# Zelana-Labs/zelana

Hardware: AMD Instinct MI355X
Metric: BN254 G1 MSM Mpoint-scalar/s + L2 proofs/sec at 1/2/4/8 MI355X (higher is better)
Workload: dtype u32

## Files before the change

zelana_amd/csrc/msm.hip:

```cpp
#include <stdarg.h>
#include <stdlib.h>
#include <stdio.h>
#include <string.h>

#include <algorithm>
#include <string>
#include <type_traits>
#include <vector>
#include <chrono>

#include "dev_io.h"
#include "ec.h"
#include "zkmi_internal.h"

namespace zk {

#define ZK_TAIL_WAVE() __builtin_amdgcn_s_setprio(3)

struct G1T {
  using F = FqOps;
  using P = FqP;
  static constexpr int CW = 8;
  static constexpr int PW = 16;
};
// ... 153 lines not shown
  extern __shared__ uint32_t hist[];
  for (uint32_t x = threadIdx.x; x < NH; x += RS_THREADS) hist[x] = 0;
  __syncthreads();
  const uint64_t base = (uint64_t)blockIdx.x * C1;
  const double inv_ne = 1.0 / (double)ne;
  constexpr int U = 8;
  for (uint32_t k0 = 0; k0 < C1; k0 += U * RS_THREADS) {
    int32_t d[U];
#pragma unroll
    for (int u = 0; u < U; u++) {
      uint64_t e = base + k0 + u * RS_THREADS + threadIdx.x;
      d[u] = (k0 + u * RS_THREADS + threadIdx.x < C1 && e < M) ? digits[e] : 0;
    }
#pragma unroll
    for (int u = 0; u < U; u++) {
      if (d[u] == 0) continue;
      uint32_t w, i;
      rs_divmod(base + k0 + u * RS_THREADS + threadIdx.x, ne, inv_ne, w, i);
      atomicAdd(&hist[(w * B + (uint32_t)(d[u] < 0 ? -d[u] : d[u]) - 1) >> lob], 1u);
    }
  }
  __syncthreads();
  for (uint32_t x = threadIdx.x; x < NH; x += RS_THREADS) cnt1[(size_t)x * nc1 + blockIdx.x] = hist[x];
}


template <int T = RS_THREADS>
__device__ __forceinline__ uint32_t rs_block_scan(const uint32_t* hist, uint32_t* lstart, uint32_t nb, uint32_t* tmp) {
  uint32_t sum = 0;
  for (uint32_t x = threadIdx.x; x < nb; x += T) sum += hist[x];
  const uint32_t lane = threadIdx.x & 63, wid = threadIdx.x >> 6;
  uint32_t inc = sum;
#pragma unroll
  for (int off = 1; off < 64; off <<= 1) {
    uint32_t t = __shfl_up(inc, off, 64);
    if (lane >= (unsigned)off) inc += t;
  }
  if (lane == 63) tmp[wid] = inc;
  __syncthreads();
  uint32_t run = inc - sum, total = 0;
#pragma unroll
  for (int w = 0; w < T / 64; w++) {
    const uint32_t tw = tmp[w];
    if ((uint32_t)w < wid) run += tw;
    total += tw;
  }
  for (uint32_t x = threadIdx.x; x < nb; x += T) {
    lstart[x] = run;
    run += hist[x];
  }
  return total;
}

template <int PER, class Fill, class Bin, bool WRITE_KEY, int T = RS_THREADS, class KT = uint32_t>
__device__ __forceinline__ void rs_scatter_core(uint32_t nsub, uint32_t nb, uint32_t* lds, Fill fill, Bin bin,
                                                 KT* __restrict__ okey, uint32_t* __restrict__ oval) {
  uint32_t* hist = lds;
  uint32_t* lstart = lds + nb;
  uint32_t* gbase = lds + 2 * nb;
  uint32_t* tmp = lds + 3 * nb;
  uint32_t* skey = tmp + T;
  uint32_t* sval = skey + PER * T;
  for (uint32_t x = threadIdx.x; x < nb; x += T) hist[x] = 0;
  __syncthreads();
  for (uint32_t sub = 0; sub < nsub; sub++) {
    uint32_t key[PER], val[PER], rk[PER];
    bool ok[PER];
    fill(sub, key, val, ok);
#pragma unroll
    for (int k = 0; k < PER; k++)
      if (ok[k]) rk[k] = atomicAdd(&hist[bin(key[k])], 1u);
    __syncthreads();
    const uint32_t total = rs_block_scan<T>(hist, lstart, nb, tmp);
    __syncthreads();
#pragma unroll
    for (int k = 0; k < PER; k++) {
      if (ok[k]) {
        uint32_t lp = lstart[bin(key[k])] + rk[k];
        skey[lp] = key[k];
        sval[lp] = val[k];
      }
    }
    __syncthreads();
    for (uint32_t q = threadIdx.x; q < total; q += T) {
      uint32_t kk = skey[q], bn = bin(kk);
      uint32_t g = gbase[bn] + (q - lstart[bn]);
      if (WRITE_KEY) okey[g] = (KT)kk;
      oval[g] = sval[q];
    }
    __syncthreads();
    for (uint32_t x = threadIdx.x; x < nb; x += T) {
      gbase[x] += hist[x];
      hist[x] = 0;
    }
    __syncthreads();
  }
}

template <int RS_ST, class Load, class Bin, bool WRITE_KEY, int T = RS_THREADS>
__device__ __forceinline__ void rs_scatter_tiles(uint32_t count, uint32_t nb, uint32_t* lds, Load load, Bin bin,
                                                 uint32_t* __restrict__ okey, uint32_t* __restrict__ oval) {
  constexpr int PER = RS_ST / T;
  auto fill = [&](uint32_t sub, uint32_t* key, uint32_t* val, bool* ok) {
#pragma unroll
    for (int k = 0; k < PER; k++) {
      const uint32_t e = sub * RS_ST + k * T + threadIdx.x;
      ok[k] = e < count && load(e, key[k], val[k]);
    }
  };
  rs_scatter_core<PER, decltype(fill), Bin, WRITE_KEY, T>((count + RS_ST - 1) / RS_ST, nb, lds, fill, bin, okey, oval);
}

__host__ __device__ constexpr size_t rs_scatter_lds(uint32_t nb, uint32_t st, uint32_t t = RS_THREADS) {
  return (3 * (size_t)nb + t + 2 * st) * 4;
}

template <int RS_ST>
__global__ void __launch_bounds__(RS_THREADS) k_rs_p1_scatter(const int32_t* __restrict__ digits, uint64_t M,
                                                              uint32_t ne, uint32_t B, uint32_t NH, uint32_t lob,
                                                              uint32_t C1, uint32_t nc1, const uint32_t* __restrict__ offs1,
                                                              uint32_t* __restrict__ okey, uint32_t* __restrict__ oval) {
  ZK_TAIL_WAVE();
  extern __shared__ uint32_t lds[];
  for (uint32_t x = threadIdx.x; x < NH; x += RS_THREADS) lds[2 * NH + x] = offs1[(size_t)x * nc1 + blockIdx.x];
  const uint64_t base = (uint64_t)blockIdx.x * C1;
  const uint32_t count = (uint32_t)std::min<uint64_t>(C1, M - base);
  auto load = [&](uint32_t e, uint32_t& key, uint32_t& val) { return rs_key(digits, base + e, ne, B, key, val); };
  auto bin = [lob](uint32_t key) { return key >> lob; };
  rs_scatter_tiles<RS_ST, decltype(load), decltype(bin), true>(count, NH, lds, load, bin, okey, oval);
}

template <int C, bool BAL>
__device__ __forceinline__ void rs_scalar_keys(const uint32_t* __restrict__ scalars, size_t i, size_t n, int Wp,
                                               uint32_t B, uint32_t* key, uint32_t* val, bool* ok, uint32_t wsel) {
  constexpr int W = msm_windows(C);
  int32_t d[W];
  scalar_digits<C, BAL>(scalars, i, d);
  const uint32_t w0 = wsel & 0xFFFFu, wn = wsel >> 16;
  uint32_t j = 0, wq = 0;
#pragma unroll
  for (int w = 0; w < W; w++) {
    const int32_t v = d[w];
    const uint32_t wr = (uint32_t)w - w0;
    ok[w] = v != 0 && (wn == 0 || wr < wn);
    key[w] = (wn ? wr : wq) * B + (uint32_t)(v < 0 ? -v : v) - 1;
    val[w] = (uint32_t)(j * n + i) | (v < 0 ? 0x80000000u : 0u);
    if (++wq == (uint32_t)Wp) {
      wq = 0;
      j++;
    }
  }
}

constexpr size_t SMALL_SORT_MAX = (size_t)1 << 18;
template <int C, bool BAL, bool BAT = false>
__global__ void __launch_bounds__(256) k_ss_count(const uint32_t* __restrict__ scalars, size_t n, int Wp, uint32_t B,
                                                  uint32_t wsel, uint32_t* __restrict__ cnt, size_t sstride = 0) {
  ZK_TAIL_WAVE();
  constexpr int W = msm_windows(C);
  const size_t i = blockIdx.x * (size_t)blockDim.x + threadIdx.x;
  if (i >= n) return;
  uint32_t key[W], val[W];
  bool ok[W];
  if (BAT) scalars += (size_t)blockIdx.y * sstride;
  rs_scalar_keys<C, BAL>(scalars, i, n, Wp, B, key, val, ok, wsel);
  const uint32_t koff = BAT ? blockIdx.y * (uint32_t)Wp * B : 0u;
#pragma unroll
// ... 246 lines not shown
template <int C, int T, bool BAL, bool BAT = false>
__global__ void __launch_bounds__(T) k_bs_scatter1(const uint32_t* __restrict__ scalars, size_t n, int Wp, uint32_t B,
                                                   uint32_t wsel, uint32_t NH, uint32_t lob, uint32_t CS, uint32_t scs,
                                                   const uint32_t* __restrict__ bintot,
                                                   const uint32_t* __restrict__ sctot,
                                                   const uint32_t* __restrict__ choff, BsKey* __restrict__ okey,
                                                   uint32_t* __restrict__ oval, uint32_t nfb = 0, size_t sstride = 0) {
  ZK_TAIL_WAVE();
  extern __shared__ uint32_t lds[];
  constexpr int W = msm_windows(C);
  uint32_t* gbase = lds + 2 * NH;
  block_prefix<T>(NH, [&](uint32_t k) { return bintot[k]; }, gbase, lds + 3 * NH);
  const uint32_t s0 = blockIdx.x >> scs;
  for (uint32_t x = threadIdx.x; x < NH; x += T) {
    uint32_t g = gbase[x] + choff[(size_t)blockIdx.x * NH + x];
    for (uint32_t q = 0; q < s0; q++) g += sctot[(size_t)q * NH + x];
    gbase[x] = g;
  }
  const uint32_t bq = BAT ? blockIdx.x / nfb : 0u;
  const size_t base = (size_t)(BAT ? blockIdx.x - bq * nfb : blockIdx.x) * CS;
  const uint32_t cnt = (uint32_t)std::min<size_t>(CS, n - base);
  const uint32_t koff = BAT ? bq * (uint32_t)Wp * B : 0u;
  if (BAT) scalars += (size_t)bq * sstride;
  auto fill = [&](uint32_t sub, uint32_t* key, uint32_t* val, bool* ok) {
    const uint32_t k = sub * T + threadIdx.x;
    if (k < cnt) {
      rs_scalar_keys<C, BAL>(scalars, base + k, n, Wp, B, key, val, ok, wsel);
      if (BAT) {
#pragma unroll
        for (int w = 0; w < W; w++) key[w] += koff;
      }
    } else {
#pragma unroll
      for (int w = 0; w < W; w++) ok[w] = false;
    }
  };
  auto bin = [lob](uint32_t key) { return key >> lob; };
  rs_scatter_core<W, decltype(fill), decltype(bin), true, T>((cnt + T - 1) / T, NH, lds, fill, bin, okey, oval);
}

__device__ __forceinline__ uint32_t bs_tiles(const uint32_t* __restrict__ bintot, uint32_t NH, uint32_t C2,
                                             uint32_t* pre, uint32_t* tst, uint32_t* tmp) {
  const uint32_t M = block_prefix<256>(NH, [&](uint32_t k) { return bintot[k]; }, pre, tmp);
  const uint32_t TT = block_prefix<256>(
      NH, [&](uint32_t k) { return max(1u, (bintot[k] + C2 - 1) / C2); }, tst, tmp);
  if (threadIdx.x == 0) {
    pre[NH] = M;
    tst[NH] = TT;
  }
  __syncthreads();
  return TT;
}

__global__ void __launch_bounds__(256) k_bs_count2(const BsKey* __restrict__ okey,
                                                   const uint32_t* __restrict__ bintot, uint32_t NH, uint32_t lob,
                                                   uint32_t C2, uint32_t T2max, uint32_t* __restrict__ thist) {
  ZK_TAIL_WAVE();
  extern __shared__ uint32_t lds[];
  const uint32_t NLO = 1u << lob, mask = NLO - 1;
  uint32_t* hist = lds;
  uint32_t* pre = lds + NLO;
  uint32_t* tst = pre + NH + 1;
  uint32_t* tmp = tst + NH + 1;
  const uint32_t t = rs_xcd_tile(blockIdx.x, T2max);
  if (t >= T2max) return;
  const uint32_t TT = bs_tiles(bintot, NH, C2, pre, tst, tmp);
  if (t >= TT) return;
  const uint32_t h = rs_tile_bin(tst, NH, t), q = t - tst[h];
  const uint32_t lo = pre[h] + q * C2, hi = min(lo + C2, pre[h + 1]);
  for (uint32_t x = threadIdx.x; x < NLO; x += 256) hist[x] = 0;
  __syncthreads();
  constexpr int U = 8;
  for (uint32_t p0 = lo; p0 < hi; p0 += U * 256) {
    uint32_t kk[U];
#pragma unroll
    for (int u = 0; u < U; u++) {
      const uint32_t p = p0 + u * 256 + threadIdx.x;
      kk[u] = p < hi ? okey[p] : 0xFFFFFFFFu;
    }
#pragma unroll
    for (int u = 0; u < U; u++)
      if (kk[u] != 0xFFFFFFFFu) atomicAdd(&hist[kk[u] & mask], 1u);
  }
  __syncthreads();
  for (uint32_t x = threadIdx.x; x < NLO; x += 256) thist[(size_t)t * NLO + x] = hist[x];
}

struct ItemsOut {
  uint4* items;
  uint32_t nmain, cap;
  uint32_t* itc;
  uint4* split;
  uint4* stage;
  uint32_t* ghist;
};

template <int ST, bool ITEMS>
__global__ void __launch_bounds__(256) k_bs_scatter2(const BsKey* __restrict__ okey,
                                                     const uint32_t* __restrict__ oval,
                                                     const uint32_t* __restrict__ bintot, uint32_t NH, uint32_t lob,
                                                     uint32_t C2, uint32_t T2max, uint32_t K,
                                                     const uint32_t* __restrict__ thist,
                                                     uint32_t* __restrict__ sval, uint32_t* __restrict__ bstart,
                                                     ItemsOut io) {
  ZK_TAIL_WAVE();
  constexpr int T = 256;
  extern __shared__ uint32_t lds[];
  const uint32_t NLO = 1u << lob, mask = NLO - 1;
  uint32_t* lstart = lds + NLO;
  uint32_t* gbase = lds + 2 * NLO;
  uint32_t* tmp = lds + 3 * NLO;
  uint32_t* skey = tmp + T;
  uint32_t* pre = skey + 2 * ST;
  uint32_t* tst = pre + NH + 1;
  const uint32_t t = rs_xcd_tile(blockIdx.x, T2max);
  if (t >= T2max) return;
  const uint32_t TT = bs_tiles(bintot, NH, C2, pre, tst, tmp);
  if (t >= TT) return;
  const uint32_t h = rs_tile_bin(tst, NH, t), q = t - tst[h];
  const uint32_t lo = pre[h] + q * C2, hi = min(lo + C2, pre[h + 1]);
  const uint32_t k0 = h * NLO;
  uint32_t* ksz = lds;
  {
    const uint32_t t0 = tst[h], nt = tst[h + 1] - t0;
    for (uint32_t x = threadIdx.x; x < NLO; x += T) {
      uint32_t tot = 0, before = 0;
      for (uint32_t qq = 0; qq < nt; qq++) {
        const uint32_t v = thist[(size_t)(t0 + qq) * NLO + x];
        before += qq < q ? v : 0u;
        tot += v;
      }
      ksz[x] = k0 + x < K ? tot : 0u;
      gbase[x] = before;
    }
    __syncthreads();
  }
  auto ksize = [&](uint32_t x) { return ksz[x]; };
  block_prefix<T>(NLO, ksize, lstart, tmp);
  if (q == 0) {
    for (uint32_t x = threadIdx.x; x < NLO; x += T)
      if (k0 + x < K) bstart[k0 + x] = pre[h] + lstart[x];
    if (h == NH - 1 && threadIdx.x == 0) bstart[K] = pre[NH];
    if constexpr (ITEMS) {
      const uint32_t cap = io.cap;
      uint32_t* ch = skey;
      uint32_t* cstart = skey + ST;
      for (uint32_t c = threadIdx.x; c <= cap; c += T) ch[c] = 0;
      __syncthreads();
      constexpr uint32_t PERX = 2048 / T;
      uint32_t tk[PERX];
#pragma unroll
      for (uint32_t j = 0; j < PERX; j++) {
        const uint32_t x = j * T + threadIdx.x;
        if (x < NLO) tk[j] = atomicAdd(&ch[min(ksize(x), cap)], 1u);
      }
      __syncthreads();
      block_prefix<T>(cap + 1, [&](uint32_t k) { return ch[cap - k]; }, cstart, tmp);
#pragma unroll
      for (uint32_t j = 0; j < PERX; j++) {
        const uint32_t x = j * T + threadIdx.x;
        if (x >= NLO) continue;
        const uint32_t size = ksize(x), cls = min(size, cap);
        const uint32_t rank = cstart[cap - cls] + tk[j];
        const uint32_t start = pre[h] + lstart[x];
        const uint32_t np = (size + cap - 1) / cap;
        uint32_t slot0 = 0xFFFFFFFFu;
        if (np > 1) {
          slot0 = atomicAdd(&io.itc[1], np);
          const uint32_t ov = atomicAdd(&io.itc[0], np - 1);
          io.split[atomicAdd(&io.itc[2], 1u)] = make_uint4(k0 + x, slot0, np, 0);
          for (uint32_t pc = 1; pc < np; pc++)
            io.items[io.nmain + ov + pc - 1] =
                make_uint4(start + pc * cap, min(start + (pc + 1) * cap, start + size), k0 + x, slot0 + pc);
        }
        io.stage[(size_t)h * NLO + rank] = make_uint4(start, start + cls, k0 + x, slot0);
      }
      for (uint32_t c = threadIdx.x; c <= cap; c += T)
        if (ch[c]) atomicAdd(&io.ghist[c], ch[c]);
      __syncthreads();
    }
  }
  for (uint32_t x = threadIdx.x; x < NLO; x += T) gbase[x] += pre[h] + lstart[x];
  auto load = [&](uint32_t e, uint32_t& key, uint32_t& val) {
    key = okey[lo + e];
    val = oval[lo + e];
    return true;
  };
  auto bin = [mask](uint32_t key) { return key & mask; };
  rs_scatter_tiles<ST, decltype(load), decltype(bin), false, T>(hi - lo, NLO, lds, load, bin, nullptr, sval);
}

__global__ void __launch_bounds__(256) k_scan_blocks(const uint32_t* in, uint32_t K, uint32_t* out,
                                                     uint32_t* __restrict__ block_sums) {
  ZK_TAIL_WAVE();
  __shared__ uint32_t sh[256];
  uint32_t base = blockIdx.x * 1024 + threadIdx.x * 4;
  uint32_t v[4], s = 0;
#pragma unroll
  for (int k = 0; k < 4; k++) {
    v[k] = base + k < K ? in[base + k] : 0;
    s += v[k];
  }
  sh[threadIdx.x] = s;
  __syncthreads();
  for (int off = 1; off < 256; off <<= 1) {
    uint32_t t = threadIdx.x >= (unsigned)off ? sh[threadIdx.x - off] : 0;
    __syncthreads();
    sh[threadIdx.x] += t;
    __syncthreads();
  }
  uint32_t excl = sh[threadIdx.x] - s;
#pragma unroll
  for (int k = 0; k < 4; k++) {
    if (base + k < K) out[base + k] = excl;
    excl += v[k];
  }
  if (threadIdx.x == 255) block_sums[blockIdx.x] = sh[255];
}
__global__ void __launch_bounds__(1024) k_scan_top(uint32_t* __restrict__ bs, uint32_t nb, uint32_t* __restrict__ total) {
  ZK_TAIL_WAVE();
  __shared__ uint32_t sh[1024];
  uint32_t carry = 0;
  for (uint32_t base = 0; base < nb; base += 1024) {
    uint32_t i = base + threadIdx.x;
    uint32_t v = i < nb ? bs[i] : 0;
    sh[threadIdx.x] = v;
    __syncthreads();
    for (int off = 1; off < 1024; off <<= 1) {
      uint32_t t = threadIdx.x >= (unsigned)off ? sh[threadIdx.x - off] : 0;
      __syncthreads();
      sh[threadIdx.x] += t;
      __syncthreads();
    }
    if (i < nb) bs[i] = sh[threadIdx.x] - v + carry;
    uint32_t blk_total = sh[1023];
    __syncthreads();
    carry += blk_total;
  }
  if (threadIdx.x == 0) *total = carry;
}
__global__ void __launch_bounds__(256) k_scan_add(uint32_t* __restrict__ out, uint32_t K,
                                                  const uint32_t* __restrict__ bs, uint32_t* __restrict__ cursor) {
// ... 1497 lines not shown
  uint32_t B, K;
  int w0 = 0;
  uint32_t wsel = 0;
  int nb = 1;
  bool batch = false;
  size_t sstride = 0;
  int Wp() const { return wsel ? msm_windows(c) : W / nb; }
};
static MsmPlan msm_plan(const zkmi_ctx* ctx, const zkmi_bases* tb, size_t n) {
  MsmPlan P;
  const bool table = tb->tc > 0 && (ctx->msm_window == 0 || ctx->msm_window == tb->tc);
  P.c = table ? tb->tc : (ctx->msm_window > 0 ? ctx->msm_window : pick_window(n));
  P.p = table ? tb->tp : 1;
  P.W = table ? tb->tw : msm_windows(P.c);
  P.bal = table && tb->tbal;
  P.ne = (size_t)P.p * n;
  P.Mmax = (size_t)P.W * P.ne;
  P.B = 1u << (P.c - 1);
  P.K = (uint32_t)P.W * P.B;
  P.bb = P.c - 1;
  P.lb = (P.bb + 1) / 2;
  P.hb = P.bb - P.lb;
  return P;
}
static MsmPlan msm_plan_batch(const zkmi_ctx* ctx, const zkmi_bases* tb, size_t n, int nb, size_t sstride) {
  MsmPlan P = msm_plan(ctx, tb, n);
  P.batch = true;
  P.nb = nb;
  P.sstride = sstride;
  P.W *= nb;
  P.K *= (uint32_t)nb;
  P.Mmax *= (size_t)nb;
  return P;
}
static bool same_plan(const MsmPlan& a, const MsmPlan& b) {
  return a.c == b.c && a.p == b.p && a.W == b.W && a.bal == b.bal;
}
static bool items_plan(const MsmPlan& P) {
  return P.K >= ITEMS_MIN_K && P.c >= 12 && P.c <= 22 && (P.W <= 2 || P.Mmax <= (size_t)64 * P.K);
}
static uint32_t item_cap(const zkmi_ctx* ctx, const MsmPlan& P) {
  const size_t share = P.Mmax / ((size_t)ctx->num_cus * 768 * 2);
  uint32_t cap = 64;
  while (cap < share && cap < ITEM_CAP_MAX) cap <<= 1;
  return cap;
}
struct BsGeom {
  uint32_t lob, NLO, NH, CS, nf, scs, C2, T2max;
  uint32_t nfb;
  size_t nmain;
  size_t ctr_words() const { return (size_t)NH + 16 + (size_t)BS_NSC * NH + 2 * (ITEM_CAP_MAX + 1); }
  uint32_t* ghist(uint32_t* ctr) const { return ctr + NH + 16 + (size_t)BS_NSC * NH; }
};
static BsGeom bs_geom(const MsmPlan& P, size_t n) {
  BsGeom g;
  uint32_t kb = 0;
  while ((1u << kb) < P.K) kb++;
  g.lob = kb >= 15 ? std::min(11u, kb) : std::max(6u, kb > 4 ? kb - 4 : 0u);
  g.NLO = 1u << g.lob;
  g.NH = (P.K + g.NLO - 1) >> g.lob;
  g.CS = 1024u * (uint32_t)std::max<size_t>(1, (n + 1024ull * 2048 - 1) / (1024ull * 2048));
  g.nfb = (uint32_t)std::max<size_t>(1, (n + g.CS - 1) / g.CS);
  g.nf = g.nfb * (uint32_t)P.nb;
  g.scs = 0;
  while (((size_t)g.nf + (1u << g.scs) - 1) >> g.scs > BS_NSC) g.scs++;
  const size_t C2B = P.Mmax < ((size_t)1 << 22) ? 4096 : 16384;
  g.C2 = (uint32_t)(C2B * std::max<size_t>(1, (P.Mmax + C2B * C2B - 1) / (C2B * C2B)));
  g.T2max = (uint32_t)((P.Mmax + g.C2 - 1) / g.C2) + g.NH;
  g.nmain = (size_t)g.NH * g.NLO;
  return g;
}
constexpr int BS_ST = 4096;
static size_t bs_lds_scatter2(const BsGeom& g) { return rs_scatter_lds(g.NLO, BS_ST, 256) + (2 * (size_t)g.NH + 2) * 4; }

template <int C, bool BAL>
static void launch_bs_p1(hipStream_t st, const uint32_t* sc, size_t n, int Wp, uint32_t B, uint32_t wsel, const BsGeom& g,
                         uint32_t* ctr, uint32_t* next_ctr, uint32_t* choff, uint32_t* okey, uint32_t* oval,
                         bool scatter, bool batch, size_t sstride) {
  constexpr int W = msm_windows(C);
  uint32_t* bintot = ctr;
  uint32_t* sctot = ctr + g.NH + 16;
  if (batch) {
    if (scatter)
      k_bs_scatter1<C, 256, BAL, true><<<g.nf, 256, rs_scatter_lds(g.NH, 256 * W, 256), st>>>(
          sc, n, Wp, B, wsel, g.NH, g.lob, g.CS, g.scs, bintot, sctot, choff, reinterpret_cast<BsKey*>(okey), oval,
          g.nfb, sstride);
    else
      k_bs_count<C, BAL, true><<<g.nf, 256, g.NH * 4, st>>>(sc, n, Wp, B, wsel, g.NH, g.lob, g.CS, g.scs, bintot,
                                                            sctot, choff, next_ctr, (uint32_t)g.ctr_words(), g.nfb,
                                                            sstride);
    return;
  }
  if (scatter)
    k_bs_scatter1<C, 256, BAL><<<g.nf, 256, rs_scatter_lds(g.NH, 256 * W, 256), st>>>(
        sc, n, Wp, B, wsel, g.NH, g.lob, g.CS, g.scs, bintot, sctot, choff, reinterpret_cast<BsKey*>(okey), oval);
  else
    k_bs_count<C, BAL><<<g.nf, 256, g.NH * 4, st>>>(sc, n, Wp, B, wsel, g.NH, g.lob, g.CS, g.scs, bintot, sctot, choff,
                                                    next_ctr, (uint32_t)g.ctr_words());
}
static int bs_p1(int c, bool bal, hipStream_t st, const uint32_t* sc, size_t n, int Wp, uint32_t B, uint32_t wsel, const BsGeom& g,
                 uint32_t* ctr, uint32_t* next_ctr, uint32_t* choff, uint32_t* okey, uint32_t* oval, bool scatter,
                 bool batch = false, size_t sstride = 0) {
  switch (c) {
#define ZK_C(CC)                                                                                  \
  case CC:                                                                                        \
    if (bal) launch_bs_p1<CC, true>(st, sc, n, Wp, B, wsel, g, ctr, next_ctr, choff, okey, oval, scatter, batch, sstride); \
    else launch_bs_p1<CC, false>(st, sc, n, Wp, B, wsel, g, ctr, next_ctr, choff, okey, oval, scatter, batch, sstride);    \
    break;
    ZK_C(12) ZK_C(13) ZK_C(14) ZK_C(15) ZK_C(16) ZK_C(17) ZK_C(18) ZK_C(19) ZK_C(20) ZK_C(21) ZK_C(22)
#undef ZK_C
    default:
      set_error("bin sort: unsupported MSM window %d", c);
      return ZKMI_EINVAL;
  }
  return 0;
}

static int debug_skip() {
#ifdef ZK_DEBUG_ABLATE
  static const int v = [] {
    const char* e = getenv("ZKMI_DEBUG_SKIP");
    return e ? atoi(e) : 0;
  }();
  return v;
#else
  return 0;
#endif
}

static int msm_sort_phase(zkmi_ctx* ctx, MsmLane* lane, const MsmPlan& P, const uint32_t* d_scalars, size_t n,
                          uint32_t** out_sval, uint32_t** out_bstart) {
  hipStream_t st = lane->st;
  Workspace& ws = lane->ws;
  uint32_t kb = 0;
  while ((1u << kb) < P.K) kb++;
  const uint32_t lob = kb > 20 ? kb - 10 : kb > 16 ? kb - 8 : 8;
  const uint32_t NH = (P.K + (1u << lob) - 1) >> lob;
  const size_t Mmax = P.Mmax;
  const uint32_t C1 = 16384u * (uint32_t)std::max<size_t>(1, (Mmax + 16384ull * 2048 - 1) / (16384ull * 2048));
  const uint32_t nc1 = (uint32_t)((Mmax + C1 - 1) / C1);
  const uint32_t C2b = std::max(8192u, 4u << lob);
  const uint32_t C2 = C2b * (uint32_t)std::max<size_t>(1, (Mmax + (size_t)C2b * 8192 - 1) / ((size_t)C2b * 8192));
  const uint32_t T2max = (uint32_t)((Mmax + C2 - 1) / C2) + NH;
  const size_t len1 = (size_t)NH * nc1, len2 = (size_t)T2max << lob;
  int32_t* digits;
  uint32_t *bstart, *sval, *cnt1, *okey, *oval, *binstart, *tstart, *cnt2, *bsums, *tot;
  const bool fused = P.c >= 12 && P.c <= 22;
  digits = nullptr;
  if (!fused) ZK_TRY(ws.get("msm_digits", Mmax * 4, (void**)&digits));
  ZK_TRY(ws.get("msm_bstart", (size_t)(P.K + 1) * 4, (void**)&bstart));
  ZK_TRY(ws.get("msm_sval", Mmax * 4, (void**)&sval));
  const bool small = fused && Mmax <= SMALL_SORT_MAX && !items_plan(P) && P.K <= (1u << 16);
  if (!small) {
    ZK_TRY(ws.get("msm_okey", Mmax * 4, (void**)&okey));
    ZK_TRY(ws.get("msm_oval", Mmax * 4, (void**)&oval));
  }
  if (ctx->msm_fork) {
    ZK_HIP(hipStreamWaitEvent(st, ctx->msm_fork, 0));
  } else {
    ZK_HIP(hipEventRecord(lane->fork, ctx->stream));
    ZK_HIP(hipStreamWaitEvent(st, lane->fork, 0));
  }
  if ((debug_skip() & 1) && lane->debug_sorted) {
    *out_sval = sval;
    *out_bstart = bstart;
    return 0;
  }
  lane->debug_sorted = 1;
  ScopedKernelTimer tm(ctx, "msm_sort", st);
  if (fused && !small) {
    const BsGeom g = bs_geom(P, n);
    const bool items = items_plan(P);
    uint32_t *ctr2, *choff, *thist;
    uint4 *it = nullptr, *split = nullptr, *stage = nullptr;
    const size_t cw = g.ctr_words();
    ZK_TRY(ws.get("msm_bs_ctr", 2 * cw * 4, (void**)&ctr2));
    if (ctr2 != lane->bs_ctr || cw != lane->bs_ctr_words || lane->bs_dirty) {
      ZK_HIP(hipMemsetAsync(ctr2, 0, 2 * cw * 4, st));
      lane->bs_ctr = ctr2;
      lane->bs_ctr_words = cw;
      lane->bs_parity = 0;
    }
    lane->bs_dirty = true;
    uint32_t* ctr = ctr2 + (size_t)lane->bs_parity * cw;
    uint32_t* next_ctr = ctr2 + (size_t)(lane->bs_parity ^ 1) * cw;
    ZK_TRY(ws.get("msm_bs_choff", (size_t)g.nf * g.NH * 4, (void**)&choff));
    ZK_TRY(ws.get("msm_bs_thist", (size_t)g.T2max * g.NLO * 4, (void**)&thist));
    ItemsOut io{nullptr, (uint32_t)g.nmain, 0, ctr + g.NH, nullptr, nullptr, g.ghist(ctr)};
    if (items) {
      io.cap = item_cap(ctx, P);
      ZK_TRY(ws.get("msm_items", (g.nmain + (Mmax + io.cap - 1) / io.cap) * 16, (void**)&it));
      ZK_TRY(ws.get("msm_split", ((Mmax + io.cap - 1) / io.cap + 1) * 16, (void**)&split));
      ZK_TRY(ws.get("msm_items_stage", g.nmain * 16, (void**)&stage));
      io.items = it;
      io.split = split;
      io.stage = stage;
    }
    ZK_TRY(bs_p1(P.c, P.bal, st, d_scalars, n, P.Wp(), P.B, P.wsel, g, ctr, next_ctr, choff, okey, oval, false, P.batch,
                 P.sstride));
    ZK_TRY(bs_p1(P.c, P.bal, st, d_scalars, n, P.Wp(), P.B, P.wsel, g, ctr, next_ctr, choff, okey, oval, true, P.batch,
                 P.sstride));
    ZK_HIP(hipEventRecord(lane->consumed, st));
    ZK_HIP(hipStreamWaitEvent(ctx->stream, lane->consumed, 0));
    const uint32_t gt = ((g.T2max + 7) / 8) * 8;
    k_bs_count2<<<gt, 256, (g.NLO + 2 * g.NH + 2 + 4) * 4, st>>>(reinterpret_cast<BsKey*>(okey), ctr, g.NH, g.lob, g.C2, g.T2max, thist);
    if (items) {
      k_bs_scatter2<BS_ST, true><<<gt, 256, bs_lds_scatter2(g), st>>>(reinterpret_cast<BsKey*>(okey), oval, ctr, g.NH, g.lob, g.C2, g.T2max,
                                                                     P.K, thist, sval, bstart, io);
      k_items_place<<<g.NH, 256, 0, st>>>(stage, g.NLO, io.cap, io.ghist, io.ghist + ITEM_CAP_MAX + 1, it,
                                          (uint32_t)g.nmain);
    } else {
      k_bs_scatter2<BS_ST, false><<<gt, 256, bs_lds_scatter2(g), st>>>(reinterpret_cast<BsKey*>(okey), oval, ctr, g.NH, g.lob, g.C2, g.T2max,
                                                                      P.K, thist, sval, bstart, io);
    }
    lane->bs_cur = ctr;
    lane->bs_parity ^= 1;
    lane->bs_dirty = false;
    ZK_HIP(hipGetLastError());
    *out_sval = sval;
    *out_bstart = bstart;
    return 0;
  }
  if (small) {
    uint32_t *scnt, *scur;
    ZK_TRY(ws.get("msm_ss_cnt", (size_t)P.K * 4, (void**)&scnt));
    ZK_TRY(ws.get("msm_ss_cursor", (size_t)P.K * 4, (void**)&scur));
    if (scnt != lane->ss_clean || P.K > lane->ss_clean_words) {
      ZK_HIP(hipMemsetAsync(scnt, 0, (size_t)P.K * 4, st));
      lane->ss_clean = scnt;
      lane->ss_clean_words = P.K;
    }
    lane->ss_clean = nullptr;
    ZK_TRY(small_sort(P.c, P.bal, st, d_scalars, n, P.Wp(), P.B, P.wsel, P.K, scnt, scur, bstart, sval,
                      P.batch ? (uint32_t)P.nb : 0u, P.sstride));
    lane->ss_clean = scnt;
    ZK_HIP(hipEventRecord(lane->consumed, st));
    ZK_HIP(hipStreamWaitEvent(ctx->stream, lane->consumed, 0));
    ZK_HIP(hipGetLastError());
    *out_sval = sval;
    *out_bstart = bstart;
    return 0;
  }
  ZK_TRY(ws.get("msm_cnt1", len1 * 4, (void**)&cnt1));
  ZK_TRY(ws.get("msm_cnt2", len2 * 4, (void**)&cnt2));
  ZK_TRY(ws.get("msm_binstart", (size_t)(NH + 1) * 4, (void**)&binstart));
  ZK_TRY(ws.get("msm_tstart", (size_t)(NH + 1) * 4, (void**)&tstart));
  ZK_TRY(ws.get("msm_bsums", ((std::max(len1, len2) + 1023) / 1024) * 4 + 16, (void**)&bsums));
  ZK_TRY(ws.get("msm_tot", 64, (void**)&tot));
  {
    ZK_TRY(dispatch_digits(P.c, st, d_scalars, n, P.p, P.batch ? P.Wp() : P.W, P.bal, digits,
                           P.batch ? (uint32_t)P.nb : 0u, P.sstride));
    ZK_HIP(hipEventRecord(lane->consumed, st));
    ZK_HIP(hipStreamWaitEvent(ctx->stream, lane->consumed, 0));
  }
  auto scan = [&](uint32_t* a, size_t len, uint32_t* total) {
    uint32_t nb = (uint32_t)((len + 1023) / 1024);
    k_scan_blocks<<<nb, 256, 0, st>>>(a, (uint32_t)len, a, bsums);
    k_scan_top<<<1, 1024, 0, st>>>(bsums, nb, total);
    k_scan_add<<<(unsigned)((len + 255) / 256), 256, 0, st>>>(a, (uint32_t)len, bsums, nullptr);
  };
  const uint32_t ne = (uint32_t)P.ne;
  k_rs_p1_count<<<nc1, RS_THREADS, NH * 4, st>>>(digits, Mmax, ne, P.B, NH, lob, C1, nc1, cnt1);
  scan(cnt1, len1, &tot[0]);
  k_rs_p1_scatter<4096><<<nc1, RS_THREADS, rs_scatter_lds(NH, 4096), st>>>(digits, Mmax, ne, P.B, NH, lob, C1, nc1,
                                                                           cnt1, okey, oval);
  k_rs_tiles<<<1, 1024, 0, st>>>(cnt1, nc1, NH, &tot[0], C2, binstart, tstart);
  const uint32_t g2 = ((T2max + 7) / 8) * 8;
// ... 50 lines not shown
  if (!job->comm) {
    job->host_words = words;
    ZK_TRY(ctx_pinned_get(ctx, words * 4, (void**)&job->host));
    job->st = st;
    ZK_HIP(hipMemcpyAsync(job->host, d_buf + SHARD_STATUS_WORDS, words * 4, hipMemcpyDeviceToHost, st));
    ZK_HIP(hipEventRecord(job->done, st));
    job->done_rec = true;
    return 0;
  }
  const int nr = job->comm->nranks;
  const bool empty = words == 0;
  k_put_words<<<1, 64, 0, st>>>(d_buf, 0u, shard_sig0(job->g2, empty ? 0 : job->c, empty ? 0 : job->bb, job->wmode),
                                empty ? 0u : (uint32_t)job->sb,
                                empty ? 0u : (uint32_t)job->W | ((uint32_t)job->w0 << 16));
  ZK_HIP(hipGetLastError());
  const size_t width = empty || job->wmode ? SHARD_PAYLOAD_WORDS : SHARD_STATUS_WORDS + words;
  if (job->comm->kind == ZKMI_COMM_RCCL) {
    uint32_t* gathered;
    ZK_TRY(lane->ws.get("msm_gathered", (size_t)nr * SHARD_PAYLOAD_WORDS * 4, (void**)&gathered));
    ZK_TRY(comm_allgather_device(job->comm, st, d_buf, gathered, SHARD_PAYLOAD_WORDS * 4));
    job->exchanged = true;
    job->host_words = width;
    ZK_TRY(ctx_pinned_get(ctx, (size_t)nr * width * 4, (void**)&job->host));
    job->st = st;
    ZK_HIP(hipMemcpy2DAsync(job->host, width * 4, gathered, SHARD_PAYLOAD_WORDS * 4, width * 4, nr,
                            hipMemcpyDeviceToHost, st));
  } else {
    job->host_words = SHARD_PAYLOAD_WORDS;
    ZK_TRY(ctx_pinned_get(ctx, SHARD_PAYLOAD_WORDS * 4, (void**)&job->host));
    job->st = st;
    ZK_HIP(hipMemcpyAsync(job->host, d_buf, width * 4, hipMemcpyDeviceToHost, st));
  }
  ZK_HIP(hipEventRecord(job->done, st));
  job->done_rec = true;
  return 0;
}

template <class G>
static int msm_acc_phase(zkmi_ctx* ctx, MsmLane* lane, const MsmPlan& P, const zkmi_bases* tb, size_t offset,
                         size_t n, const uint32_t* sval, const uint32_t* bstart, zkmi_msm_job* job) {
  constexpr int XW = 4 * G::CW;
  using GS = std::conditional_t<G::CW == 8, G1Tn, G>;
  using GB = G;
  hipStream_t st = lane->st;
  Workspace& ws = lane->ws;
  const uint32_t* d_bases = tb->d_pts + offset * G::PW;
  const uint32_t K = P.K;
  const int W = P.W, bb = P.bb, lb = P.lb, hb = P.hb;
  const size_t Mmax = P.Mmax;
  const uint32_t tn = (uint32_t)n, tskip = P.p > 1 ? (uint32_t)(tb->n - n) : 0u;
  uint32_t* buckets;
  ZK_TRY(ws.get("msm_buckets", (size_t)K * XW * 4, (void**)&buckets));
  if (items_plan(P)) {
    const BsGeom g = bs_geom(P, n);
    const uint32_t cap = item_cap(ctx, P);
    const size_t npieces = (Mmax + cap - 1) / cap;
    const size_t items_max = g.nmain + npieces;
    uint32_t* ctr = lane->bs_cur;
    uint32_t* xpts;
    uint4 *items, *split;
    ZK_TRY(ws.get("msm_items", items_max * 16, (void**)&items));
    ZK_TRY(ws.get("msm_split", (npieces + 1) * 16, (void**)&split));
    ZK_TRY(ws.get("msm_xpts", (2 * npieces + 2) * XW * 4, (void**)&xpts));
    const uint32_t* itc = ctr + g.NH;
    if (ctx->acc_last && ctx->acc_last != lane) ZK_HIP(hipStreamWaitEvent(st, ctx->acc_last->acc_done, 0));
    {
      ScopedKernelTimer tm(ctx, G::CW == 8 ? "msm_acc0_g1" : "msm_acc0_g2", st);
#ifndef ZK_ACC_VPAD_LOG
#define ZK_ACC_VPAD_LOG 27
#endif
      const bool vpad = G::CW == 8 && Mmax >= ((size_t)1 << std::min(ZK_ACC_VPAD_LOG, 63));
      auto kern = G::CW == 8 ? (vpad ? k_acc_items_g1<true> : k_acc_items_g1<false>) : k_acc_items_g2;
#ifndef ZK_ACC_LDS_B
#define ZK_ACC_LDS_B 41984
#endif
      const size_t acc_lds = G::CW == 8 && !vpad ? (size_t)ZK_ACC_LDS_B : 0;
      kern<<<(unsigned)((items_max + 255) / 256), 256, acc_lds, st>>>(
          items, &itc[0], (uint32_t)g.nmain, sval, d_bases, tn, tskip, buckets, xpts);
    }
    ZK_HIP(hipEventRecord(lane->acc_done, st));
    ctx->acc_last = lane;
    ScopedKernelTimer tm(ctx, "msm_accN", st);
    auto comb = K <= CUTSUM_COOP_K ? k_split_combine<GS> : k_split_combine<GB>;
    const size_t maxsplit = std::min<size_t>(K, npieces / 2 + 1);
    comb<<<(unsigned)std::min<size_t>((maxsplit + 3) / 4, 1024), 256, 0, st>>>(split, &itc[2], xpts, buckets);
    ZK_HIP(hipGetLastError());
  } else {
    uint32_t *flags, *xkey, *xvalid, *xpts, *ykey, *yvalid, *ypts;
    ZK_TRY(ws.get("msm_flags", 64 * 4, (void**)&flags));
    const size_t tpc = 1024;
    const size_t acc_threads = (size_t)ctx->num_cus * tpc;
    uint32_t L = (uint32_t)std::max<size_t>(4, (Mmax + acc_threads - 1) / acc_threads);
    uint32_t nch = (uint32_t)((Mmax + L - 1) / L);
    const size_t xl = 2 * (size_t)nch + 1;
    ZK_TRY(ws.get("msm_xkey", xl * 4 + 64, (void**)&xkey));
    ZK_TRY(ws.get("msm_xvalid", xl * 4 + 64, (void**)&xvalid));
    ZK_TRY(ws.get("msm_xpts", (xl + 2) * XW * 4, (void**)&xpts));
    ZK_TRY(ws.get("msm_ykey", xl * 4 + 64, (void**)&ykey));
    ZK_TRY(ws.get("msm_yvalid", xl * 4 + 64, (void**)&yvalid));
    ZK_TRY(ws.get("msm_ypts", (xl + 2) * XW * 4, (void**)&ypts));
    {
      ScopedKernelTimer tm(ctx, G::CW == 8 ? "msm_acc0_g1" : "msm_acc0_g2", st);
      Acc0Kernel<G>::fn<<<(nch + 255) / 256, 256, 0, st>>>(sval, bstart, K, L, nch, d_bases, tn, tskip, buckets, xkey,
                                                            xvalid, xpts, flags);
      ZK_HIP(hipGetLastError());
    }
    ScopedKernelTimer tm(ctx, "msm_accN", st);
// ... 502 lines not shown
```

Before: 936.9.

## Split bucket-sort rank from scatter, fit tiles to CUs, stage 16-bit keys

The second-pass bucket sort used to compute bucket starts and item lists inside the scatter kernel, guarded by a q==0 tile check. That work now runs in a separate per-bin rank kernel, and the scatter kernel reads bstart to build its own bases. Tile assignment to blocks is rebalanced per XCD, and C2 is resized so the tile count fits about three blocks per CU. Split-piece item writes are spread across the wavefront with a ballot loop, and LDS staging keys shrink to 16 bits to cut shared-memory use. This adds one kernel launch and relies on low-order keys fitting in 16 bits.

```diff
diff --git a/zelana_amd/csrc/msm.hip b/zelana_amd/csrc/msm.hip
--- a/zelana_amd/csrc/msm.hip
+++ b/zelana_amd/csrc/msm.hip
@@ -229,15 +229,17 @@
   return total;
 }
 
-template <int PER, class Fill, class Bin, bool WRITE_KEY, int T = RS_THREADS, class KT = uint32_t>
+template <int PER, class Fill, class Bin, bool WRITE_KEY, int T = RS_THREADS, class KT = uint32_t, class SK = uint32_t>
 __device__ __forceinline__ void rs_scatter_core(uint32_t nsub, uint32_t nb, uint32_t* lds, Fill fill, Bin bin,
                                                  KT* __restrict__ okey, uint32_t* __restrict__ oval) {
+  static_assert(sizeof(SK) == 4 || !WRITE_KEY, "written keys are staged whole");
+  static_assert((PER * T * sizeof(SK)) % 4 == 0, "sval stays word-aligned");
   uint32_t* hist = lds;
   uint32_t* lstart = lds + nb;
   uint32_t* gbase = lds + 2 * nb;
   uint32_t* tmp = lds + 3 * nb;
-  uint32_t* skey = tmp + T;
-  uint32_t* sval = skey + PER * T;
+  SK* skey = reinterpret_cast<SK*>(tmp + T);
+  uint32_t* sval = reinterpret_cast<uint32_t*>(skey + PER * T);
   for (uint32_t x = threadIdx.x; x < nb; x += T) hist[x] = 0;
   __syncthreads();
   for (uint32_t sub = 0; sub < nsub; sub++) {
@@ -254,7 +256,7 @@
     for (int k = 0; k < PER; k++) {
       if (ok[k]) {
         uint32_t lp = lstart[bin(key[k])] + rk[k];
-        skey[lp] = key[k];
+        skey[lp] = (SK)key[k];
         sval[lp] = val[k];
       }
     }
@@ -274,7 +276,7 @@
   }
 }
 
-template <int RS_ST, class Load, class Bin, bool WRITE_KEY, int T = RS_THREADS>
+template <int RS_ST, class Load, class Bin, bool WRITE_KEY, int T = RS_THREADS, class SK = uint32_t>
 __device__ __forceinline__ void rs_scatter_tiles(uint32_t count, uint32_t nb, uint32_t* lds, Load load, Bin bin,
                                                  uint32_t* __restrict__ okey, uint32_t* __restrict__ oval) {
   constexpr int PER = RS_ST / T;
@@ -285,11 +287,13 @@
       ok[k] = e < count && load(e, key[k], val[k]);
     }
   };
-  rs_scatter_core<PER, decltype(fill), Bin, WRITE_KEY, T>((count + RS_ST - 1) / RS_ST, nb, lds, fill, bin, okey, oval);
-}
-
-__host__ __device__ constexpr size_t rs_scatter_lds(uint32_t nb, uint32_t st, uint32_t t = RS_THREADS) {
-  return (3 * (size_t)nb + t + 2 * st) * 4;
+  rs_scatter_core<PER, decltype(fill), Bin, WRITE_KEY, T, uint32_t, SK>((count + RS_ST - 1) / RS_ST, nb, lds, fill, bin,
+                                                                        okey, oval);
+}
+
+__host__ __device__ constexpr size_t rs_scatter_lds(uint32_t nb, uint32_t st, uint32_t t = RS_THREADS,
+                                                    uint32_t key_bytes = 4) {
+  return (3 * (size_t)nb + t) * 4 + (size_t)st * (key_bytes + 4);
 }
 
 template <int RS_ST>
@@ -642,6 +646,24 @@
   return TT;
 }
 
+#ifndef ZK_BS_FIT
+#define ZK_BS_FIT 1
+#endif
+constexpr uint32_t BS_NOTILE = 0xFFFFFFFFu;
+__device__ __forceinline__ uint32_t bs_my_tile(const uint32_t* __restrict__ bintot, uint32_t NH, uint32_t C2,
+                                               uint32_t T2max, uint32_t* pre, uint32_t* tst, uint32_t* tmp) {
+#if ZK_BS_FIT
+  const uint32_t TT = bs_tiles(bintot, NH, C2, pre, tst, tmp);
+  const uint32_t per = (TT + 7) / 8, r = blockIdx.x >> 3;
+  const uint32_t t = r < per ? (blockIdx.x & 7) * per + r : BS_NOTILE;
+  return t < TT ? t : BS_NOTILE;
+#else
+  const uint32_t t = rs_xcd_tile(blockIdx.x, T2max);
+  if (t >= T2max) return BS_NOTILE;
+  return t < bs_tiles(bintot, NH, C2, pre, tst, tmp) ? t : BS_NOTILE;
+#endif
+}
+
 __global__ void __launch_bounds__(256) k_bs_count2(const BsKey* __restrict__ okey,
                                                    const uint32_t* __restrict__ bintot, uint32_t NH, uint32_t lob,
                                                    uint32_t C2, uint32_t T2max, uint32_t* __restrict__ thist) {
@@ -652,10 +674,8 @@
   uint32_t* pre = lds + NLO;
   uint32_t* tst = pre + NH + 1;
   uint32_t* tmp = tst + NH + 1;
-  const uint32_t t = rs_xcd_tile(blockIdx.x, T2max);
-  if (t >= T2max) return;
-  const uint32_t TT = bs_tiles(bintot, NH, C2, pre, tst, tmp);
-  if (t >= TT) return;
+  const uint32_t t = bs_my_tile(bintot, NH, C2, T2max, pre, tst, tmp);
+  if (t == BS_NOTILE) return;
   const uint32_t h = rs_tile_bin(tst, NH, t), q = t - tst[h];
   const uint32_t lo = pre[h] + q * C2, hi = min(lo + C2, pre[h + 1]);
   for (uint32_t x = threadIdx.x; x < NLO; x += 256) hist[x] = 0;
@@ -685,56 +705,45 @@
   uint32_t* ghist;
 };
 
-template <int ST, bool ITEMS>
-__global__ void __launch_bounds__(256) k_bs_scatter2(const BsKey* __restrict__ okey,
-                                                     const uint32_t* __restrict__ oval,
-                                                     const uint32_t* __restrict__ bintot, uint32_t NH, uint32_t lob,
-                                                     uint32_t C2, uint32_t T2max, uint32_t K,
-                                                     const uint32_t* __restrict__ thist,
-                                                     uint32_t* __restrict__ sval, uint32_t* __restrict__ bstart,
-                                                     ItemsOut io) {
+__host__ __device__ constexpr size_t bs_rank_lds(uint32_t NLO, uint32_t NH, uint32_t cap, bool rank) {
+  return (2 * (size_t)NLO + 2 * (size_t)NH + 2 + 4 + (rank ? 2 * ((size_t)cap + 1) : 0)) * 4;
+}
+
+template <bool RANK>
+__global__ void __launch_bounds__(256) k_bs_rank(const uint32_t* __restrict__ bintot, uint32_t NH, uint32_t lob,
+                                                 uint32_t C2, uint32_t K, const uint32_t* __restrict__ thist,
+                                                 uint32_t* __restrict__ bstart, ItemsOut io) {
   ZK_TAIL_WAVE();
   constexpr int T = 256;
   extern __shared__ uint32_t lds[];
-  const uint32_t NLO = 1u << lob, mask = NLO - 1;
+  const uint32_t NLO = 1u << lob;
+  uint32_t* ksz = lds;
   uint32_t* lstart = lds + NLO;
-  uint32_t* gbase = lds + 2 * NLO;
-  uint32_t* tmp = lds + 3 * NLO;
-  uint32_t* skey = tmp + T;
-  uint32_t* pre = skey + 2 * ST;
+  uint32_t* pre = lds + 2 * NLO;
   uint32_t* tst = pre + NH + 1;
-  const uint32_t t = rs_xcd_tile(blockIdx.x, T2max);
-  if (t >= T2max) return;
-  const uint32_t TT = bs_tiles(bintot, NH, C2, pre, tst, tmp);
-  if (t >= TT) return;
-  const uint32_t h = rs_tile_bin(tst, NH, t), q = t - tst[h];
-  const uint32_t lo = pre[h] + q * C2, hi = min(lo + C2, pre[h + 1]);
+  uint32_t* tmp = tst + NH + 1;
+  const uint32_t h = blockIdx.x;
+  bs_tiles(bintot, NH, C2, pre, tst, tmp);
   const uint32_t k0 = h * NLO;
-  uint32_t* ksz = lds;
   {
     const uint32_t t0 = tst[h], nt = tst[h + 1] - t0;
     for (uint32_t x = threadIdx.x; x < NLO; x += T) {
-      uint32_t tot = 0, before = 0;
-      for (uint32_t qq = 0; qq < nt; qq++) {
-        const uint32_t v = thist[(size_t)(t0 + qq) * NLO + x];
-        before += qq < q ? v : 0u;
-        tot += v;
-      }
+      uint32_t tot = 0;
+      for (uint32_t qq = 0; qq < nt; qq++) tot += thist[(size_t)(t0 + qq) * NLO + x];
       ksz[x] = k0 + x < K ? tot : 0u;
-      gbase[x] = before;
     }
     __syncthreads();
   }
   auto ksize = [&](uint32_t x) { return ksz[x]; };
   block_prefix<T>(NLO, ksize, lstart, tmp);
-  if (q == 0) {
+  {
     for (uint32_t x = threadIdx.x; x < NLO; x += T)
       if (k0 + x < K) bstart[k0 + x] = pre[h] + lstart[x];
     if (h == NH - 1 && threadIdx.x == 0) bstart[K] = pre[NH];
-    if constexpr (ITEMS) {
+    if constexpr (RANK) {
       const uint32_t cap = io.cap;
-      uint32_t* ch = skey;
-      uint32_t* cstart = skey + ST;
+      uint32_t* ch = tmp + 4;
+      uint32_t* cstart = ch + cap + 1;
       for (uint32_t c = threadIdx.x; c <= cap; c += T) ch[c] = 0;
       __syncthreads();
       constexpr uint32_t PERX = 2048 / T;
@@ -754,30 +763,67 @@
         const uint32_t rank = cstart[cap - cls] + tk[j];
         const uint32_t start = pre[h] + lstart[x];
         const uint32_t np = (size + cap - 1) / cap;
-        uint32_t slot0 = 0xFFFFFFFFu;
+        uint32_t slot0 = 0xFFFFFFFFu, ov = 0;
         if (np > 1) {
           slot0 = atomicAdd(&io.itc[1], np);
-          const uint32_t ov = atomicAdd(&io.itc[0], np - 1);
+          ov = atomicAdd(&io.itc[0], np - 1);
           io.split[atomicAdd(&io.itc[2], 1u)] = make_uint4(k0 + x, slot0, np, 0);
-          for (uint32_t pc = 1; pc < np; pc++)
-            io.items[io.nmain + ov + pc - 1] =
-                make_uint4(start + pc * cap, min(start + (pc + 1) * cap, start + size), k0 + x, slot0 + pc);
         }
         io.stage[(size_t)h * NLO + rank] = make_uint4(start, start + cls, k0 + x, slot0);
+        for (uint64_t m = __ballot(np > 1); m; m &= m - 1) {
+          const int src = __ffsll((unsigned long long)m) - 1;
+          const uint32_t s_start = __shfl(start, src, 64), s_end = s_start + __shfl(size, src, 64);
+          const uint32_t s_key = __shfl(k0 + x, src, 64), s_slot = __shfl(slot0, src, 64);
+          const uint32_t s_ov = __shfl(ov, src, 64), s_np = __shfl(np, src, 64);
+          for (uint32_t pc = 1 + (threadIdx.x & 63); pc < s_np; pc += 64)
+            io.items[io.nmain + s_ov + pc - 1] =
+                make_uint4(s_start + pc * cap, min(s_start + (pc + 1) * cap, s_end), s_key, s_slot + pc);
+        }
       }
       for (uint32_t c = threadIdx.x; c <= cap; c += T)
         if (ch[c]) atomicAdd(&io.ghist[c], ch[c]);
-      __syncthreads();
-    }
-  }
-  for (uint32_t x = threadIdx.x; x < NLO; x += T) gbase[x] += pre[h] + lstart[x];
+    }
+  }
+}
+
+#ifndef ZK_BS_SKEY16
+#define ZK_BS_SKEY16 1
+#endif
+using BsStageKey = std::conditional_t<ZK_BS_SKEY16 != 0, uint16_t, uint32_t>;
+
+template <int ST>
+__global__ void __launch_bounds__(256) k_bs_scatter2(const BsKey* __restrict__ okey,
+                                                     const uint32_t* __restrict__ oval,
+                                                     const uint32_t* __restrict__ bintot, uint32_t NH, uint32_t lob,
+                                                     uint32_t C2, uint32_t T2max, uint32_t K,
+                                                     const uint32_t* __restrict__ thist,
+                                                     const uint32_t* __restrict__ bstart,
+                                                     uint32_t* __restrict__ sval) {
+  ZK_TAIL_WAVE();
+  constexpr int T = 256;
+  extern __shared__ uint32_t lds[];
+  const uint32_t NLO = 1u << lob, mask = NLO - 1;
+  uint32_t* gbase = lds + 2 * NLO;
+  uint32_t* tmp = lds + 3 * NLO;
+  uint32_t* pre = tmp + T + ST * (sizeof(BsStageKey) + 4) / 4;
+  uint32_t* tst = pre + NH + 1;
+  const uint32_t t = bs_my_tile(bintot, NH, C2, T2max, pre, tst, tmp);
+  if (t == BS_NOTILE) return;
+  const uint32_t h = rs_tile_bin(tst, NH, t), q = t - tst[h];
+  const uint32_t lo = pre[h] + q * C2, hi = min(lo + C2, pre[h + 1]);
+  const uint32_t k0 = h * NLO, t0 = tst[h];
+  for (uint32_t x = threadIdx.x; x < NLO; x += T) {
+    uint32_t g = k0 + x < K ? bstart[k0 + x] : 0u;
+    for (uint32_t qq = 0; qq < q; qq++) g += thist[(size_t)(t0 + qq) * NLO + x];
+    gbase[x] = g;
+  }
   auto load = [&](uint32_t e, uint32_t& key, uint32_t& val) {
     key = okey[lo + e];
     val = oval[lo + e];
     return true;
   };
   auto bin = [mask](uint32_t key) { return key & mask; };
-  rs_scatter_tiles<ST, decltype(load), decltype(bin), false, T>(hi - lo, NLO, lds, load, bin, nullptr, sval);
+  rs_scatter_tiles<ST, decltype(load), decltype(bin), false, T, BsStageKey>(hi - lo, NLO, lds, load, bin, nullptr, sval);
 }
 
 __global__ void __launch_bounds__(256) k_scan_blocks(const uint32_t* in, uint32_t K, uint32_t* out,
@@ -2381,7 +2427,8 @@
   size_t ctr_words() const { return (size_t)NH + 16 + (size_t)BS_NSC * NH + 2 * (ITEM_CAP_MAX + 1); }
   uint32_t* ghist(uint32_t* ctr) const { return ctr + NH + 16 + (size_t)BS_NSC * NH; }
 };
-static BsGeom bs_geom(const MsmPlan& P, size_t n) {
+constexpr int BS_ST = 4096;
+static BsGeom bs_geom(const MsmPlan& P, size_t n, int cus) {
   BsGeom g;
   uint32_t kb = 0;
   while ((1u << kb) < P.K) kb++;
@@ -2395,12 +2442,20 @@
   while (((size_t)g.nf + (1u << g.scs) - 1) >> g.scs > BS_NSC) g.scs++;
   const size_t C2B = P.Mmax < ((size_t)1 << 22) ? 4096 : 16384;
   g.C2 = (uint32_t)(C2B * std::max<size_t>(1, (P.Mmax + C2B * C2B - 1) / (C2B * C2B)));
+#if ZK_BS_FIT
+  const size_t slots = (size_t)cus * 3;
+  if (C2B == 16384 && P.Mmax / g.C2 + g.NH < 4 * slots && g.NH <= slots) {
+    const size_t subs = (P.Mmax / g.NH + P.Mmax / g.NH / 32 + BS_ST - 1) / BS_ST, per_bin = slots / g.NH;
+    g.C2 = (uint32_t)(BS_ST * std::max<size_t>(1, (subs + per_bin - 1) / per_bin));
+  }
+#endif
   g.T2max = (uint32_t)((P.Mmax + g.C2 - 1) / g.C2) + g.NH;
   g.nmain = (size_t)g.NH * g.NLO;
   return g;
 }
-constexpr int BS_ST = 4096;
-static size_t bs_lds_scatter2(const BsGeom& g) { return rs_scatter_lds(g.NLO, BS_ST, 256) + (2 * (size_t)g.NH + 2) * 4; }
+static size_t bs_lds_scatter2(const BsGeom& g) {
+  return rs_scatter_lds(g.NLO, BS_ST, 256, sizeof(BsStageKey)) + (2 * (size_t)g.NH + 2) * 4;
+}
 
 template <int C, bool BAL>
 static void launch_bs_p1(hipStream_t st, const uint32_t* sc, size_t n, int Wp, uint32_t B, uint32_t wsel, const BsGeom& g,
@@ -2498,7 +2553,7 @@
   lane->debug_sorted = 1;
   ScopedKernelTimer tm(ctx, "msm_sort", st);
   if (fused && !small) {
-    const BsGeom g = bs_geom(P, n);
+    const BsGeom g = bs_geom(P, n, ctx->num_cus);
     const bool items = items_plan(P);
     uint32_t *ctr2, *choff, *thist;
     uint4 *it = nullptr, *split = nullptr, *stage = nullptr;
@@ -2534,14 +2589,16 @@
     const uint32_t gt = ((g.T2max + 7) / 8) * 8;
     k_bs_count2<<<gt, 256, (g.NLO + 2 * g.NH + 2 + 4) * 4, st>>>(reinterpret_cast<BsKey*>(okey), ctr, g.NH, g.lob, g.C2, g.T2max, thist);
     if (items) {
-      k_bs_scatter2<BS_ST, true><<<gt, 256, bs_lds_scatter2(g), st>>>(reinterpret_cast<BsKey*>(okey), oval, ctr, g.NH, g.lob, g.C2, g.T2max,
-                                                                     P.K, thist, sval, bstart, io);
+      k_bs_rank<true><<<g.NH, 256, bs_rank_lds(g.NLO, g.NH, io.cap, true), st>>>(ctr, g.NH, g.lob, g.C2, P.K, thist,
+                                                                                 bstart, io);
       k_items_place<<<g.NH, 256, 0, st>>>(stage, g.NLO, io.cap, io.ghist, io.ghist + ITEM_CAP_MAX + 1, it,
                                           (uint32_t)g.nmain);
     } else {
-      k_bs_scatter2<BS_ST, false><<<gt, 256, bs_lds_scatter2(g), st>>>(reinterpret_cast<BsKey*>(okey), oval, ctr, g.NH, g.lob, g.C2, g.T2max,
-                                                                      P.K, thist, sval, bstart, io);
-    }
+      k_bs_rank<false><<<g.NH, 256, bs_rank_lds(g.NLO, g.NH, 0, false), st>>>(ctr, g.NH, g.lob, g.C2, P.K, thist,
+                                                                              bstart, io);
+    }
+    k_bs_scatter2<BS_ST><<<gt, 256, bs_lds_scatter2(g), st>>>(reinterpret_cast<BsKey*>(okey), oval, ctr, g.NH, g.lob,
+                                                              g.C2, g.T2max, P.K, thist, bstart, sval);
     lane->bs_cur = ctr;
     lane->bs_parity ^= 1;
     lane->bs_dirty = false;
@@ -2698,7 +2755,7 @@
   uint32_t* buckets;
   ZK_TRY(ws.get("msm_buckets", (size_t)K * XW * 4, (void**)&buckets));
   if (items_plan(P)) {
-    const BsGeom g = bs_geom(P, n);
+    const BsGeom g = bs_geom(P, n, ctx->num_cus);
     const uint32_t cap = item_cap(ctx, P);
     const size_t npieces = (Mmax + cap - 1) / cap;
     const size_t items_max = g.nmain + npieces;
```

Result: no change. 935.3, median of 2 (-0.2%).
